# ashual/scene_generation

Hardware: AMD Instinct MI355X
Metric: images/sec G+D step, 128x128 <=8-obj scene graphs (higher is better)
Workload: dtype f32

## Files before the change

### scene_generation_amd/csrc/common.h

```cpp
#pragma once
#include <hip/hip_runtime.h>
#include <stdint.h>
#include <stdio.h>
#include <atomic>
#include "../../include/sg2im_hip.h"

#define SG_WAVE 64

void sg_set_error(const char* fmt, ...);
int sg_check_indices_if_enabled(const int64_t* idx, int64_t n, int64_t lo, int64_t hi, const char* what, hipStream_t s);

#define SG_ARG_CHECK(cond, ...)                 \
  do {                                          \
    if (!(cond)) {                              \
      sg_set_error(__VA_ARGS__);                \
      return -1;                                \
    }                                           \
  } while (0)

#define SG_LAUNCH_CHECK(name)                                               \
  do {                                                                      \
    hipError_t e__ = hipGetLastError();                                     \
    if (e__ != hipSuccess) {                                                \
      sg_set_error("%s: launch failed: %s", name, hipGetErrorString(e__)); \
      return (int)e__;                                                      \
    }                                                                       \
  } while (0)

enum SgOpt {
  SG_OPT_TILE,
  SG_OPT_T128_MIN,
  SG_OPT_TILE3,
  SG_OPT_TILE3_MIN,
  SG_OPT_SPLIT_TARGET,
  SG_OPT_SPLIT_KMIN,
  SG_OPT_SPLITS,
  SG_OPT_FIXEDTAP,
  SG_OPT_WINO_WT,
  SG_OPT_W24_SMALL,
  SG_OPT_W24_S,
  SG_OPT_W24_PMIN,
  SG_OPT_WINO_ADJOINT,
  SG_OPT_WINO24,
  SG_OPT_LINEAR_NSUB,
  SG_OPT_LINEAR_SKINNY,
  SG_OPT_WGRAD_ROWSUM,
  SG_OPT_LAYOUT_REG,
  SG_OPT_LAYOUT_DSPLIT,
  SG_OPT_BN_BLOCKS,
  SG_OPT_INSTNORM_REG,
  SG_OPT_WGRAD_XCD,
  SG_OPT_WINO_REUSE,
  SG_OPT_WINO_FOLD_CELLS,
  SG_OPT_WINO_PIPE,
  SG_OPT_CHECK_INDICES,
  SG_OPT_LAST_BLOCK,
  SG_OPT_WINO_GEMM_TILE,
  SG_OPT_WINO43,
  SG_OPT_GCONV_FUSED_GATHER,
  SG_OPT_W24_GEMM_TILE,
  SG_OPT_WINO_IN_FUSE,
  SG_OPT_W43_NSUB,
  SG_OPT_W43_KFOLD,
  SG_OPT_WAVE_PRIO,
  SG_OPT_PAR_XCD_CHUNK,
  SG_OPT_W43_TAIL_SPLIT,
  SG_OPT_TAIL_SMAX,
  SG_OPT_TAIL_KTMIN,
  SG_OPT_W43_WGRAD_TILE,
  SG_OPT_PAR_SPLIT,
  SG_OPT_TAIL_CAPTURE,
  SG_OPT_WGRAD_PADDED,
  SG_OPT_COUNT
};
extern std::atomic<int> g_sg_opt[SG_OPT_COUNT];
static inline int sg_opt(int id) { return g_sg_opt[id].load(std::memory_order_relaxed); }
extern FILE* g_sg_launch_log;

enum {
  SG_K_IGEMM_BASE = 0, SG_K_IGEMM_COUNT = 48,
  SG_K_LINEAR = 48, SG_K_LAYOUT_FWD, SG_K_LAYOUT_BWD, SG_K_INSTNORM, SG_K_BATCHNORM, SG_K_ADAM, SG_K_SEGSUM,
  SG_K_CROP, SG_K_OTHER,
  SG_K_WINO_GEMM_128, SG_K_WINO_GEMM_64, SG_K_WINO_XFORM,
  SG_K_HEAD,
  SG_K_INSTNORM_BWD,
  SG_K_WINO24_GEMM,
  SG_K_WINO43_GEMM,
  SG_K_LAYOUT_TEST_PLANES,
  SG_K_DEPROCESS,
  SG_K_LAYOUT_RGB,
  SG_K_KMEANS_ASSIGN, SG_K_KMEANS_UPDATE, SG_K_KMEANS_RELOCATE, SG_K_KMEANS_PP,
  SG_K_SCENEGRAPH_CENTERS, SG_K_SCENEGRAPH_DERIVE, SG_K_SCENEGRAPH_AGREE,
  SG_K_MAXPOOL3S2, SG_K_ADD_RELU, SG_K_BN_FOLD, SG_K_SGD, SG_K_CLASSIFY_STATS,
  SG_K_RECT_CONV_T64, SG_K_RECT_CONV_T32, SG_K_RECT_CONV_T64W, SG_K_RECT_REDUCE, SG_K_INCEPTION_POOL, SG_K_RESIZE_BILINEAR,
  SG_K_SOFTMAX_ROWS, SG_K_INCEPTION_SCORE,
  SG_K_COUNT
};
static inline int sg_igemm_kind(int family, int KS, int tile) {
  const int k = KS == 1 ? 0 : (KS == 3 ? 1 : (KS == 4 ? 2 : 3));
  return SG_K_IGEMM_BASE + family * 16 + k * 4 + tile;
}
extern int g_sg_prof_on;
void sg_prof_begin(int kind, hipStream_t s);
void sg_prof_end(int kind, hipStream_t s, double flops, double bytes);

struct SgProfScope {
  int kind; hipStream_t s; double flops, bytes; bool on;
  SgProfScope(int k, hipStream_t st, double f, double b) : kind(k), s(st), flops(f), bytes(b), on(g_sg_prof_on != 0) {
    if (on) sg_prof_begin(kind, s);
  }
  ~SgProfScope() { if (on) sg_prof_end(kind, s, flops, bytes); }
};

struct FastDiv {
  unsigned m, s, d;
  FastDiv() : m(0), s(0), d(1) {}
  explicit FastDiv(unsigned dd) : m(0), s(0), d(dd) {
    if (dd > 1) {
      unsigned sh = 0;
      while ((1u << sh) < dd) ++sh;
      m = (unsigned)((((uint64_t)1) << (31 + sh)) / dd + 1);
      s = sh - 1;
    }
  }
  __device__ __forceinline__ unsigned div(unsigned n) const { return d == 1 ? n : (__umulhi(n, m) >> s); }
};

static inline int sg_cdiv(int64_t a, int64_t b) { return (int)((a + b - 1) / b); }

__device__ __forceinline__ float sg_apply_act(float v, int act, float slope) {
  switch (act) {
    case SG_ACT_RELU: return v > 0.f ? v : 0.f;
    case SG_ACT_LEAKY: return v > 0.f ? v : v * slope;
    case SG_ACT_TANH: return tanhf(v);
    case SG_ACT_SIGMOID: return 1.f / (1.f + expf(-v));
    default: return v;
  }
}

__device__ __forceinline__ float sg_wave_sum(float v) {
#pragma unroll
  for (int o = 32; o > 0; o >>= 1) v += __shfl_xor(v, o, 64);
  return v;
}

__device__ __forceinline__ float sg_sum_strided(const float* __restrict__ p, size_t stride, int S) {
  float v = 0.f;
  for (int z0 = 0; z0 < S; z0 += 8) {
    float t[8];
#pragma unroll
    for (int e = 0; e < 8; ++e) t[e] = z0 + e < S ? p[(size_t)(z0 + e) * stride] : 0.f;
#pragma unroll
    for (int e = 0; e < 8; ++e)
      if (z0 + e < S) v += t[e];
  }
  return v;
}

__device__ __forceinline__ void sg_publish(float* p, float v) { __hip_atomic_store(p, v, __ATOMIC_RELAXED, __HIP_MEMORY_SCOPE_AGENT); }
__device__ __forceinline__ float sg_consume(const float* p) {
  return __hip_atomic_load(const_cast<float*>(p), __ATOMIC_RELAXED, __HIP_MEMORY_SCOPE_AGENT);
}
__device__ __forceinline__ bool sg_arrive_last(int* counter, int narrive, int* flag) {
  asm volatile("s_waitcnt vmcnt(0)" ::: "memory");
  __syncthreads();
  if (threadIdx.x == 0 && threadIdx.y == 0 && threadIdx.z == 0) {
    const int t = __hip_atomic_fetch_add(counter, 1, __ATOMIC_RELAXED, __HIP_MEMORY_SCOPE_AGENT);
    const int last = t == narrive - 1;
    if (last) __hip_atomic_store(counter, 0, __ATOMIC_RELAXED, __HIP_MEMORY_SCOPE_AGENT);
    *flag = last;
  }
  __syncthreads();
  return *flag != 0;
}
int* sg_counter_alloc(hipStream_t s, int n = 1, bool always = false, int family = 1);
float* sg_tail_scratch(hipStream_t s, size_t bytes);

__device__ __forceinline__ float sg_block_sum(float v, float* red) {
  const int lane = threadIdx.x & 63, wid = threadIdx.x >> 6, nw = (blockDim.x + 63) >> 6;
  v = sg_wave_sum(v);
  __syncthreads();
  if (lane == 0) red[wid] = v;
  __syncthreads();
  float t = 0.f;
  for (int i = 0; i < nw; ++i) t += red[i];
  return t;
}
```

### scene_generation_amd/csrc/layout.hip

```cpp
#include "common.h"
#include <stdlib.h>

namespace {

__device__ __forceinline__ float lin01(int j, int n) {
  if (n == 1) return 0.f;
  const float step = 1.f / (float)(n - 1);
  return j < n / 2 ? step * (float)j : 1.f - step * (float)(n - 1 - j);
}
__device__ __forceinline__ float lin10(int j, int n) {
  if (n == 1) return 1.f;
  const float step = -1.f / (float)(n - 1);
  return j < n / 2 ? 1.f + step * (float)j : 0.f - step * (float)(n - 1 - j);
}

struct Tap { int i0, i1; float w0, w1; };

__device__ __forceinline__ float tap_coord(float g, int size, int ac) {
  return ac ? (g + 1.f) * 0.5f * (float)(size - 1) : ((g + 1.f) * (float)size - 1.f) * 0.5f;
}
__device__ __forceinline__ Tap make_tap(float g, int size, int ac = 0) {
  Tap t;
  const float p = tap_coord(g, size, ac);
  if (!(fabsf(p) < 1e8f)) {
// ... 510 lines not shown
  const int max_fit = (int)(budget / per_obj);
  SG_ARG_CHECK(max_fit >= 1, "sg_masks_to_layout_fwd: D=%d too large for LDS", D);
  if (cap > max_fit) cap = max_fit;
  const size_t lds_bytes = (size_t)cap * per_obj;
  SgProfScope prof(SG_K_LAYOUT_FWD, s, 0, 4.0 * N * D * (double)H * W + 4.0 * O * D + (masks_i64 ? 8.0 : 4.0) * O * M * M);
  const int regform = sg_opt(SG_OPT_LAYOUT_REG);
  if (regform && use_vec == 4 && (size_t)D * 12 * sizeof(float) <= 64 * 1024) {
    const int tiles = sg_cdiv(H * W, 1024);
    int dsplit = sg_opt(SG_OPT_LAYOUT_DSPLIT);
    dsplit = dsplit < 1 ? 1 : (dsplit > 8 ? 8 : dsplit);
    if (dsplit > D / 16) dsplit = D / 16 > 0 ? D / 16 : 1;
    const int dchunk = sg_cdiv(D, dsplit);
    const dim3 g4(tiles, N, sg_cdiv(D, dchunk));
    const size_t lds = (size_t)dchunk * 12 * sizeof(float);
    if (masks_i64) hipLaunchKernelGGL((layout_fwd_reg_kernel<true, 12>), g4, dim3(256), lds, s, vecs, boxes, masks, seg_off, out, D, M, H, W, avg, g_align_corners, dchunk);
    else hipLaunchKernelGGL((layout_fwd_reg_kernel<false, 12>), g4, dim3(256), lds, s, vecs, boxes, masks, seg_off, out, D, M, H, W, avg, g_align_corners, dchunk);
    SG_LAUNCH_CHECK("sg_masks_to_layout_fwd");
    return 0;
  }
  const dim3 grid(sg_cdiv(H * W, 256 * use_vec), N);
#define LAUNCH_LAYOUT(I64, VEC)                                                                                         \
  do {                                                                                                                 \
    hipFuncSetAttribute(reinterpret_cast<const void*>(&layout_fwd_kernel<I64, VEC>),                                    \
                        hipFuncAttributeMaxDynamicSharedMemorySize, (int)lds_bytes);                                    \
    hipLaunchKernelGGL((layout_fwd_kernel<I64, VEC>), grid, dim3(256), lds_bytes, s, vecs, boxes, masks, seg_off, out, \
                       D, M, H, W, avg, cap, g_align_corners);                                                          \
  } while (0)
  if (masks_i64) { if (use_vec == 4) LAUNCH_LAYOUT(true, 4); else LAUNCH_LAYOUT(true, 1); }
  else { if (use_vec == 4) LAUNCH_LAYOUT(false, 4); else LAUNCH_LAYOUT(false, 1); }
#undef LAUNCH_LAYOUT
  SG_LAUNCH_CHECK("sg_masks_to_layout_fwd");
  return 0;
}

extern "C" size_t sg_masks_to_layout_test_ws_bytes(int O) { return (size_t)(O > 0 ? O : 1) * (sizeof(double) + sizeof(int32_t)) + 16; }

extern "C" int sg_masks_to_layout_test_fwd(const float* vecs, const float* boxes, const void* masks, int masks_i64,
                                           const int32_t* seg_off, float* out, void* ws, size_t ws_bytes, int N, int O, int D,
                                           int M, int H, int W, int avg, sgStream stream) {
  SG_ARG_CHECK(vecs && boxes && masks && seg_off && out && ws && N > 0 && O > 0 && D > 0 && M > 0 && H > 0 && W > 0,
               "sg_masks_to_layout_test_fwd: bad arguments");
  SG_ARG_CHECK(ws_bytes >= sg_masks_to_layout_test_ws_bytes(O), "sg_masks_to_layout_test_fwd: workspace too small");
  hipStream_t s = (hipStream_t)stream;
  double* mass = reinterpret_cast<double*>(ws);
  int32_t* order = reinterpret_cast<int32_t*>(mass + O);
  SgProfScope prof(SG_K_LAYOUT_FWD, s, 0, 4.0 * N * D * (double)H * W);
  const dim3 grid(sg_cdiv(H * W, 256), N);
  if (masks_i64) {
    hipLaunchKernelGGL((layout_mass_kernel<true>), dim3(O), dim3(256), 0, s, vecs, boxes, masks, mass, D, M, H, W, g_align_corners);
    hipLaunchKernelGGL(layout_order_kernel, dim3(N), dim3(64), 0, s, (const double*)mass, seg_off, order);
    hipLaunchKernelGGL((layout_test_fwd_kernel<true>), grid, dim3(256), 0, s, vecs, boxes, masks, seg_off,
                       (const int32_t*)order, out, D, M, H, W, avg, g_align_corners);
  } else {
    hipLaunchKernelGGL((layout_mass_kernel<false>), dim3(O), dim3(256), 0, s, vecs, boxes, masks, mass, D, M, H, W, g_align_corners);
    hipLaunchKernelGGL(layout_order_kernel, dim3(N), dim3(64), 0, s, (const double*)mass, seg_off, order);
    hipLaunchKernelGGL((layout_test_fwd_kernel<false>), grid, dim3(256), 0, s, vecs, boxes, masks, seg_off,
                       (const int32_t*)order, out, D, M, H, W, avg, g_align_corners);
  }
  SG_LAUNCH_CHECK("sg_masks_to_layout_test_fwd");
  return 0;
}

extern "C" size_t sg_masks_to_layout_test_planes_ws_bytes(int O) { return sg_masks_to_layout_test_ws_bytes(O); }

extern "C" int sg_masks_to_layout_test_planes(const float* vecs, const float* boxes, const void* masks, int masks_i64,
                                              const int32_t* seg_off, const int64_t* plane_idx, float* Z, int32_t* winner,
                                              float* value, void* ws, size_t ws_bytes, int N, int O, int D, int J, int M, int H,
                                              int W, int avg, sgStream stream) {
  SG_ARG_CHECK(vecs && boxes && masks && seg_off && plane_idx && Z && winner && ws && N > 0 && O > 0 && D > 0 && J > 0 && M > 0 &&
                   H > 0 && W > 0,
               "sg_masks_to_layout_test_planes: bad arguments");
  SG_ARG_CHECK(ws_bytes >= sg_masks_to_layout_test_planes_ws_bytes(O), "sg_masks_to_layout_test_planes: workspace too small");
  hipStream_t s = (hipStream_t)stream;
  double* mass = reinterpret_cast<double*>(ws);
  int32_t* order = reinterpret_cast<int32_t*>(mass + O);
  const int ac = g_align_corners;
  SgProfScope prof(SG_K_LAYOUT_TEST_PLANES, s, 0, 4.0 * N * (J + (value ? 2 : 1)) * (double)H * W);
  if (masks_i64) hipLaunchKernelGGL((layout_mass_kernel<true>), dim3(O), dim3(256), 0, s, vecs, boxes, masks, mass, D, M, H, W, ac);
  else hipLaunchKernelGGL((layout_mass_kernel<false>), dim3(O), dim3(256), 0, s, vecs, boxes, masks, mass, D, M, H, W, ac);
  hipLaunchKernelGGL(layout_order_kernel, dim3(N), dim3(64), 0, s, (const double*)mass, seg_off, order);
#define LAUNCH_PLANES(I64, VEC)                                                                                              \
  hipLaunchKernelGGL((layout_test_planes_kernel<I64, VEC>), dim3(sg_cdiv(H * W, 256 * VEC), N), dim3(256), 0, s, boxes, masks, \
                     seg_off, (const int32_t*)order, plane_idx, Z, winner, value, J, M, H, W, avg, ac)
  if (W % 4 == 0) { if (masks_i64) LAUNCH_PLANES(true, 4); else LAUNCH_PLANES(false, 4); }
  else { if (masks_i64) LAUNCH_PLANES(true, 1); else LAUNCH_PLANES(false, 1); }
#undef LAUNCH_PLANES
  SG_LAUNCH_CHECK("sg_masks_to_layout_test_planes");
  return 0;
}

extern "C" int sg_masks_to_layout_bwd_vecs(const float* gout, const float* boxes, const void* masks, int masks_i64,
                                           const int64_t* obj_to_img, const int32_t* seg_off, float* g_vecs, int N, int O,
                                           int D, int M, int H, int W, int avg, int d_begin, sgStream stream) {
  SG_ARG_CHECK(gout && boxes && masks && seg_off && g_vecs && N > 0 && O > 0 && D > 0 && d_begin >= 0 && d_begin < D,
               "sg_masks_to_layout_bwd_vecs: bad arguments");
  (void)obj_to_img;
  hipStream_t s = (hipStream_t)stream;
  if (d_begin > 0)
    hipLaunchKernelGGL(zero_cols_kernel, dim3(sg_cdiv((size_t)O * d_begin, 256)), dim3(256), 0, s, g_vecs, O, D, d_begin);
  SgProfScope prof(SG_K_LAYOUT_BWD, s, 0, 4.0 * N * (D - d_begin) * (double)H * W);
  const dim3 grid(D - d_begin, N);
  if (masks_i64) hipLaunchKernelGGL(layout_bwd_vecs_kernel<true>, grid, dim3(256), 0, s, gout, boxes, masks, seg_off, g_vecs, D, M, H, W, avg, d_begin, g_align_corners);
  else hipLaunchKernelGGL(layout_bwd_vecs_kernel<false>, grid, dim3(256), 0, s, gout, boxes, masks, seg_off, g_vecs, D, M, H, W, avg, d_begin, g_align_corners);
  SG_LAUNCH_CHECK("sg_masks_to_layout_bwd_vecs");
  return 0;
}

extern "C" int sg_crop_bbox_fwd(const float* feats, const float* boxes, const int64_t* box_to_feat, float* out, int N, int C,
                                int H, int W, int B, int HH, int WW, sgStream stream) {
  SG_ARG_CHECK(feats && N > 0 && C > 0 && B >= 0 && HH > 0 && WW > 0 && (B == 0 || (boxes && box_to_feat && out)),
               "sg_crop_bbox_fwd: bad arguments");
  if (B == 0) return 0;
  hipStream_t s = (hipStream_t)stream;
  SgProfScope prof(SG_K_CROP, s, 0, 4.0 * B * C * (double)HH * WW + 4.0 * N * C * (double)H * W);
  hipLaunchKernelGGL(crop_fwd_kernel, dim3(sg_cdiv((size_t)B * HH * WW, 256)), dim3(256), 0, s, feats, boxes, box_to_feat, out,
                     C, H, W, B, HH, WW, g_align_corners);
  SG_LAUNCH_CHECK("sg_crop_bbox_fwd");
  return 0;
}

extern "C" int sg_crop_bbox_bwd(const float* gout, const float* boxes, const int64_t* box_to_feat, float* g_feats, int N, int C,
                                int H, int W, int B, int HH, int WW, sgStream stream) {
  SG_ARG_CHECK(g_feats && N > 0 && C > 0 && H > 0 && W > 0 && B >= 0 && (B == 0 || (gout && boxes && box_to_feat)),
               "sg_crop_bbox_bwd: bad arguments");
  hipStream_t s = (hipStream_t)stream;
  if (B == 0) {
    if (hipMemsetAsync(g_feats, 0, (size_t)N * C * H * W * sizeof(float), s) != hipSuccess) {
      sg_set_error("sg_crop_bbox_bwd: hipMemsetAsync failed");
      return -1;
    }
    return 0;
  }
  SgProfScope prof(SG_K_CROP, s, 0, 4.0 * B * C * (double)HH * WW + 4.0 * N * C * (double)H * W);
  if (C <= 1)
    hipLaunchKernelGGL(crop_bwd_gather_kernel<1>, dim3(sg_cdiv(H * W, 256), N), dim3(256), 0, s, gout, boxes, box_to_feat,
                       g_feats, C, H, W, B, HH, WW, g_align_corners);
  else
    hipLaunchKernelGGL(crop_bwd_gather_kernel<4>, dim3(sg_cdiv(H * W, 256), N), dim3(256), 0, s, gout, boxes, box_to_feat,
                       g_feats, C, H, W, B, HH, WW, g_align_corners);
  SG_LAUNCH_CHECK("sg_crop_bbox_bwd");
  return 0;
}

struct JJTap { int i0, i1; float w0, w1; };
__device__ __forceinline__ JJTap jj_tap(float c0, float c1, int j, int n, int size) {
  const float X = (lin10(j, n) * c0 + lin01(j, n) * c1) * (float)size;
  const float hi = (float)(size - 1);
  const float f0 = fminf(fmaxf(floorf(X), 0.f), hi), f1 = fminf(fmaxf(f0 + 1.f, 0.f), hi);
  JJTap t;
  t.i0 = (int)f0; t.i1 = (int)f1; t.w0 = f1 - X; t.w1 = X - f0;
  return t;
}
__global__ void crop_jj_fwd_kernel(const float* __restrict__ feats, const float* __restrict__ boxes, float* __restrict__ out, int N,
                                   int C, int H, int W, int HH, int WW) {
  const size_t i = (size_t)blockIdx.x * blockDim.x + threadIdx.x;
  if (i >= (size_t)N * C * HH * WW) return;
  const int x = i % WW, y = (i / WW) % HH, c = (i / ((size_t)WW * HH)) % C, n = i / ((size_t)WW * HH * C);
  const JJTap tx = jj_tap(boxes[n * 4 + 0], boxes[n * 4 + 2], x, WW, W), ty = jj_tap(boxes[n * 4 + 1], boxes[n * 4 + 3], y, HH, H);
  const float* f = feats + ((size_t)n * C + c) * H * W;
  float v = (tx.w0 * ty.w0) * f[ty.i0 * W + tx.i0];
  v += (tx.w0 * ty.w1) * f[ty.i1 * W + tx.i0];
  v += (tx.w1 * ty.w0) * f[ty.i0 * W + tx.i1];
  v += (tx.w1 * ty.w1) * f[ty.i1 * W + tx.i1];
  out[i] = v;
}
__global__ void crop_jj_bwd_kernel(const float* __restrict__ gout, const float* __restrict__ boxes, float* __restrict__ gf, int N,
                                   int C, int H, int W, int HH, int WW) {
  const size_t i = (size_t)blockIdx.x * blockDim.x + threadIdx.x;
  if (i >= (size_t)N * C * H * W) return;
  const int u = i % W, r = (i / W) % H, c = (i / ((size_t)W * H)) % C, n = i / ((size_t)W * H * C);
  const float bx0 = boxes[n * 4 + 0], by0 = boxes[n * 4 + 1], bx1 = boxes[n * 4 + 2], by1 = boxes[n * 4 + 3];
  const float* g = gout + ((size_t)n * C + c) * HH * WW;
  float acc = 0.f;
  for (int y = 0; y < HH; ++y) {
    const JJTap ty = jj_tap(by0, by1, y, HH, H);
    const float wy = (ty.i0 == r ? ty.w0 : 0.f) + (ty.i1 == r ? ty.w1 : 0.f);
    if (ty.i0 != r && ty.i1 != r) continue;
    for (int x = 0; x < WW; ++x) {
      const JJTap tx = jj_tap(bx0, bx1, x, WW, W);
      if (tx.i0 != u && tx.i1 != u) continue;
      const float wx = (tx.i0 == u ? tx.w0 : 0.f) + (tx.i1 == u ? tx.w1 : 0.f);
      acc += (wx * wy) * g[y * WW + x];
    }
  }
  gf[i] = acc;
}

extern "C" int sg_crop_bbox_jj_fwd(const float* feats, const float* boxes, float* out, int N, int C, int H, int W, int HH, int WW,
                                   sgStream stream) {
  SG_ARG_CHECK(feats && boxes && out && N > 0 && C > 0 && H > 0 && W > 0 && HH > 0 && WW > 0, "sg_crop_bbox_jj_fwd: bad arguments");
  hipLaunchKernelGGL(crop_jj_fwd_kernel, dim3(sg_cdiv((size_t)N * C * HH * WW, 256)), dim3(256), 0, (hipStream_t)stream, feats, boxes,
                     out, N, C, H, W, HH, WW);
  SG_LAUNCH_CHECK("sg_crop_bbox_jj_fwd");
  return 0;
}
extern "C" int sg_crop_bbox_jj_bwd(const float* gout, const float* boxes, float* g_feats, int N, int C, int H, int W, int HH, int WW,
                                   sgStream stream) {
  SG_ARG_CHECK(gout && boxes && g_feats && N > 0 && C > 0 && H > 0 && W > 0 && HH > 0 && WW > 0, "sg_crop_bbox_jj_bwd: bad arguments");
  hipLaunchKernelGGL(crop_jj_bwd_kernel, dim3(sg_cdiv((size_t)N * C * H * W, 256)), dim3(256), 0, (hipStream_t)stream, gout, boxes,
                     g_feats, N, C, H, W, HH, WW);
  SG_LAUNCH_CHECK("sg_crop_bbox_jj_bwd");
  return 0;
}

extern "C" int sg_vector_pool_exchange(float* pool, const float* vectors, const int32_t* plan, float* out, int O, int R,
                                       int pool_size, sgStream stream) {
  SG_ARG_CHECK(pool && vectors && plan && out && O >= 0 && R > 0 && pool_size > 0, "sg_vector_pool_exchange: bad arguments");
  if (O == 0) return 0;
  hipStream_t s = (hipStream_t)stream;
  const dim3 grid(sg_cdiv((size_t)O * R, 256));
  hipLaunchKernelGGL(pool_gather_kernel, grid, dim3(256), 0, s, (const float*)pool, vectors, plan, out, O, R, pool_size);
  hipLaunchKernelGGL(pool_scatter_kernel, grid, dim3(256), 0, s, pool, vectors, plan, O, R, pool_size);
  SG_LAUNCH_CHECK("sg_vector_pool_exchange");
  return 0;
}

namespace {

__global__ void factored_weights_fwd_kernel(const float* __restrict__ W, const float* __restrict__ repr,
                                            const int64_t* __restrict__ objs, const int32_t* __restrict__ seg, float* __restrict__ wimg,
                                            int N, int M, int L, int KS2, int C, int R, int C2) {
  const size_t i = (size_t)blockIdx.x * blockDim.x + threadIdx.x;
  if (i >= (size_t)N * M * L * KS2) return;
  const int t = (int)(i % KS2);
  const int j = (int)((i / KS2) % L);
  const int m = (int)((i / ((size_t)KS2 * L)) % M);
  const int n = (int)(i / ((size_t)KS2 * L * M));
  const int cnt = seg[n + 1] - seg[n];
  const int Ct = C + R + C2;
  const float* Wm = W + (size_t)m * Ct * KS2 + t;
  float v = 0.f;
  if (j < cnt) {
    const int o = seg[n] + j;
    v = Wm[(size_t)objs[o] * KS2];
    const float* r = repr + (size_t)o * R;
    for (int d = 0; d < R; ++d) v += r[d] * Wm[(size_t)(C + d) * KS2];
  } else if (j < cnt + C2) {
    v = Wm[(size_t)(C + R + (j - cnt)) * KS2];
  }
  wimg[i] = v;
}

__global__ void factored_weights_bwd_w_kernel(const float* __restrict__ gwimg, const float* __restrict__ repr,
                                              const int64_t* __restrict__ objs, const int32_t* __restrict__ seg,
                                              const int64_t* __restrict__ img_idx, float* __restrict__ gW, int N, int O, int M,
                                              int L, int KS2, int C, int R, int C2) {
  const int Ct = C + R + C2;
  const size_t i = (size_t)blockIdx.x * blockDim.x + threadIdx.x;
  if (i >= (size_t)M * Ct * KS2) return;
  const int t = (int)(i % KS2);
  const int c = (int)((i / KS2) % Ct);
  const int m = (int)(i / ((size_t)KS2 * Ct));
  float s = 0.f;
  if (c < C + R) {
    for (int o = 0; o < O; ++o) {
      float wgt;
      if (c < C) { if ((int)objs[o] != c) continue; wgt = 1.f; }
      else wgt = repr[(size_t)o * R + (c - C)];
      const int n = (int)img_idx[o], j = o - seg[n];
      s += wgt * gwimg[(((size_t)n * M + m) * L + j) * KS2 + t];
    }
  } else {
    const int e = c - C - R;
    for (int n = 0; n < N; ++n) s += gwimg[(((size_t)n * M + m) * L + (seg[n + 1] - seg[n]) + e) * KS2 + t];
  }
  gW[i] = s;
}

__global__ void __launch_bounds__(256) factored_weights_bwd_w_lds_kernel(
    const float* __restrict__ gwimg, const float* __restrict__ repr, const int64_t* __restrict__ objs,
    const int32_t* __restrict__ seg, const int64_t* __restrict__ img_idx, float* __restrict__ gW, int N, int O, int M, int L,
    int KS2, int C, int R, int C2) {
  extern __shared__ int ws_lds[];
  int* cls = ws_lds;
  int* base = ws_lds + O;
  for (int o = threadIdx.x; o < O; o += 256) {
    const int n = (int)img_idx[o];
    cls[o] = (int)objs[o];
    base[o] = n * M * L + (o - seg[n]);
  }
  __syncthreads();
  const int Ct = C + R + C2;
  const size_t i = (size_t)blockIdx.x * blockDim.x + threadIdx.x;
  if (i >= (size_t)M * Ct * KS2) return;
  const int t = (int)(i % KS2);
  const int c = (int)((i / KS2) % Ct);
  const int m = (int)(i / ((size_t)KS2 * Ct));
  const int mL = m * L;
  float s = 0.f;
  if (c < C) {
    for (int o = 0; o < O; ++o)
      if (cls[o] == c) s += gwimg[(size_t)(base[o] + mL) * KS2 + t];
  } else if (c < C + R) {
    const float* rp = repr + (c - C);
#pragma unroll 4
    for (int o = 0; o < O; ++o) s += rp[(size_t)o * R] * gwimg[(size_t)(base[o] + mL) * KS2 + t];
  } else {
    const int e = c - C - R;
    for (int n = 0; n < N; ++n) s += gwimg[(((size_t)n * M + m) * L + (seg[n + 1] - seg[n]) + e) * KS2 + t];
  }
  gW[i] = s;
}

__global__ void __launch_bounds__(256) factored_weights_bwd_repr_kernel(const float* __restrict__ gwimg, const float* __restrict__ W,
                                                                       const int32_t* __restrict__ seg,
                                                                       const int64_t* __restrict__ img_idx,
                                                                       float* __restrict__ grepr, int O, int M, int L, int KS2,
                                                                       int C, int R, int C2) {
  const int w = blockIdx.x * 4 + (threadIdx.x >> 6), lane = threadIdx.x & 63;
  if (w >= O * R) return;
  const int o = w / R, d = w - o * R;
  const int n = (int)img_idx[o], j = o - seg[n];
  const int Ct = C + R + C2;
  float s = 0.f;
  for (int q = lane; q < M * KS2; q += 64) {
    const int m = q / KS2, t = q - m * KS2;
    s += gwimg[(((size_t)n * M + m) * L + j) * KS2 + t] * W[((size_t)m * Ct + C + d) * KS2 + t];
  }
  s = sg_wave_sum(s);
  if (lane == 0) grepr[w] = s;
}

}

extern "C" int sg_factored_weights_fwd(const float* w, const float* repr, const int64_t* objs, const int32_t* seg_off,
                                       float* wimg, int N, int O, int M, int L, int KS2, int C, int R, int C2, sgStream stream) {
  SG_ARG_CHECK(w && repr && objs && seg_off && wimg && N > 0 && O >= 0 && M > 0 && L > 0 && KS2 > 0 && C >= 0 && R >= 0 && C2 >= 0,
               "sg_factored_weights_fwd: bad arguments");
  const size_t n = (size_t)N * M * L * KS2;
  hipLaunchKernelGGL(factored_weights_fwd_kernel, dim3(sg_cdiv(n, 256)), dim3(256), 0, (hipStream_t)stream, w, repr, objs, seg_off,
                     wimg, N, M, L, KS2, C, R, C2);
  SG_LAUNCH_CHECK("sg_factored_weights_fwd");
  return 0;
}

extern "C" int sg_factored_weights_bwd(const float* gwimg, const float* w, const float* repr, const int64_t* objs,
                                       const int32_t* seg_off, const int64_t* img_idx, float* gw, float* grepr, int N, int O,
                                       int M, int L, int KS2, int C, int R, int C2, sgStream stream) {
  SG_ARG_CHECK(gwimg && w && repr && objs && seg_off && img_idx && (gw || grepr) && N > 0 && O > 0,
               "sg_factored_weights_bwd: bad arguments");
  hipStream_t s = (hipStream_t)stream;
  if (gw) {
    const size_t n = (size_t)M * (C + R + C2) * KS2;
    if (O <= 4096 && (size_t)N * M * L < (1u << 30))
      hipLaunchKernelGGL(factored_weights_bwd_w_lds_kernel, dim3(sg_cdiv(n, 256)), dim3(256), (size_t)O * 2 * sizeof(int), s, gwimg,
                         repr, objs, seg_off, img_idx, gw, N, O, M, L, KS2, C, R, C2);
    else
      hipLaunchKernelGGL(factored_weights_bwd_w_kernel, dim3(sg_cdiv(n, 256)), dim3(256), 0, s, gwimg, repr, objs, seg_off, img_idx,
                         gw, N, O, M, L, KS2, C, R, C2);
  }
  if (grepr && R > 0)
    hipLaunchKernelGGL(factored_weights_bwd_repr_kernel, dim3(sg_cdiv((size_t)O * R, 4)), dim3(256), 0, s, gwimg, w, seg_off, img_idx,
                       grepr, O, M, L, KS2, C, R, C2);
  SG_LAUNCH_CHECK("sg_factored_weights_bwd");
  return 0;
}

namespace {

__global__ void __launch_bounds__(256) layout_objmap_kernel(const float* __restrict__ gout, const float* __restrict__ vecs,
                                                           const int64_t* __restrict__ o2i, const int32_t* __restrict__ seg,
                                                           float* __restrict__ T, int D, int HW, int avg) {
  const int o = blockIdx.y;
  const int px = blockIdx.x * 256 + threadIdx.x;
  if (px >= HW) return;
  const int n = (int)o2i[o];
  const float* g = gout + (size_t)n * D * HW + px;
  const float* v = vecs + (size_t)o * D;
  float s = 0.f;
  for (int d = 0; d < D; ++d) s += g[(size_t)d * HW] * v[d];
  if (avg) { const int cnt = seg[n + 1] - seg[n]; s = s / (float)(cnt > 1 ? cnt : 1); }
  T[(size_t)o * HW + px] = s;
}

__device__ __forceinline__ void layout_axis_range(float b0, float b1, int n_pix, int M, int y, int& lo, int& hi, int ac) {
  const float p0 = tap_coord(box_coord(0.f, b0, b1), M, ac), p1 = tap_coord(box_coord(1.f, b0, b1), M, ac);
  lo = 0; hi = n_pix - 1;
  if (n_pix == 1 || !(fabsf(p0) < 1e8f) || !(fabsf(p1) < 1e8f)) return;
  const float s = (p1 - p0) / (float)(n_pix - 1);
  if (fabsf(s) < 1e-6f) return;
  float a = ((float)(y - 1) - p0) / s, b = ((float)(y + 1) - p0) / s;
  if (a > b) { const float t = a; a = b; b = t; }
  const float fl = floorf(a) - 1.f, fh = ceilf(b) + 1.f;
  lo = fl < 0.f ? 0 : (fl > (float)(n_pix - 1) ? n_pix : (int)fl);
  hi = fh > (float)(n_pix - 1) ? n_pix - 1 : (fh < 0.f ? -1 : (int)fh);
}

__global__ void __launch_bounds__(256) layout_bwd_masks_kernel(const float* __restrict__ T, const float* __restrict__ boxes,
                                                              float* __restrict__ gm, int M, int H, int W, int ac) {
  const int o = blockIdx.y;
  const int e = blockIdx.x * 256 + threadIdx.x;
  if (e >= M * M) return;
  const int y = e / M, x = e - y * M;
  const float x0 = boxes[o * 4 + 0], y0 = boxes[o * 4 + 1], x1 = boxes[o * 4 + 2], y1 = boxes[o * 4 + 3];
  int hlo, hhi, wlo, whi;
  layout_axis_range(y0, y1, H, M, y, hlo, hhi, ac);
  layout_axis_range(x0, x1, W, M, x, wlo, whi, ac);
  const float* t = T + (size_t)o * H * W;
  float s = 0.f;
  for (int h = hlo; h <= hhi; ++h) {
    const Tap ty = make_tap(box_coord(lin01(h, H), y0, y1), M, ac);
    const float wy = (ty.i0 == y ? ty.w0 : 0.f) + (ty.i1 == y ? ty.w1 : 0.f);
    if (wy == 0.f) continue;
    for (int w = wlo; w <= whi; ++w) {
      const Tap tx = make_tap(box_coord(lin01(w, W), x0, x1), M, ac);
      const float wx = (tx.i0 == x ? tx.w0 : 0.f) + (tx.i1 == x ? tx.w1 : 0.f);
      if (wx != 0.f) s += t[h * W + w] * (wy * wx);
    }
  }
  gm[(size_t)o * M * M + e] = s;
}

template <bool I64>
__global__ void __launch_bounds__(256) layout_bwd_boxes_kernel(const float* __restrict__ T, const float* __restrict__ boxes,
                                                              const void* __restrict__ masks, float* __restrict__ gb, int M, int H,
                                                              int W, int ac) {
  __shared__ float red[16];
  const size_t o = blockIdx.x;
  const float x0 = boxes[o * 4 + 0], y0 = boxes[o * 4 + 1], x1 = boxes[o * 4 + 2], y1 = boxes[o * 4 + 3];
  const float dx = x1 - x0, dy = y1 - y0;
  const float scale = ac ? 0.5f * (float)(M - 1) : 0.5f * (float)M;
  const float* t = T + o * H * W;
  float g0 = 0.f, g1 = 0.f, g2 = 0.f, g3 = 0.f;
  for (int p = threadIdx.x; p < H * W; p += 256) {
    const int h = p / W, w = p - h * W;
    const float Y = lin01(h, H), X = lin01(w, W);
    const Tap ty = make_tap(box_coord(Y, y0, y1), M, ac), tx = make_tap(box_coord(X, x0, x1), M, ac);
    const float m00 = mask_at<I64>(masks, o, M, ty.i0, tx.i0), m01 = mask_at<I64>(masks, o, M, ty.i0, tx.i1);
    const float m10 = mask_at<I64>(masks, o, M, ty.i1, tx.i0), m11 = mask_at<I64>(masks, o, M, ty.i1, tx.i1);
    const float px = tap_coord(box_coord(X, x0, x1), M, ac), py = tap_coord(box_coord(Y, y0, y1), M, ac);
    const bool fin = fabsf(px) < 1e8f && fabsf(py) < 1e8f;
    const float flx = floorf(px), fly = floorf(py);
    const float ix0 = (flx >= 0.f && flx < (float)M) ? 1.f : 0.f, ix1 = (flx + 1.f >= 0.f && flx + 1.f < (float)M) ? 1.f : 0.f;
    const float iy0 = (fly >= 0.f && fly < (float)M) ? 1.f : 0.f, iy1 = (fly + 1.f >= 0.f && fly + 1.f < (float)M) ? 1.f : 0.f;
    const float dSdx = ((m01 * ix1 - m00 * ix0) * ty.w0 + (m11 * ix1 - m10 * ix0) * ty.w1);
    const float dSdy = ((m10 * iy1 - m00 * iy0) * tx.w0 + (m11 * iy1 - m01 * iy0) * tx.w1);
    const float tv = fin ? t[p] : 0.f;
    const float cx = tv * dSdx * scale * 2.f / (dx * dx), cy = tv * dSdy * scale * 2.f / (dy * dy);
    g0 += cx * (X - x1); g2 += -cx * (X - x0);
    g1 += cy * (Y - y1); g3 += -cy * (Y - y0);
  }
  g0 = sg_block_sum(g0, red); g1 = sg_block_sum(g1, red); g2 = sg_block_sum(g2, red); g3 = sg_block_sum(g3, red);
  if (threadIdx.x == 0) { gb[o * 4 + 0] = g0; gb[o * 4 + 1] = g1; gb[o * 4 + 2] = g2; gb[o * 4 + 3] = g3; }
}

}

extern "C" size_t sg_masks_to_layout_bwd_geom_ws_bytes(int O, int H, int W) { return (size_t)(O > 0 ? O : 1) * H * W * sizeof(float); }

extern "C" int sg_masks_to_layout_bwd_geom(const float* gout, const float* vecs, const float* boxes, const void* masks, int masks_i64,
                                           const int64_t* obj_to_img, const int32_t* seg_off, float* g_masks, float* g_boxes,
                                           void* ws, size_t ws_bytes, int N, int O, int D, int M, int H, int W, int avg,
                                           sgStream stream) {
  SG_ARG_CHECK(gout && vecs && boxes && masks && obj_to_img && seg_off && ws && (g_masks || g_boxes) && N > 0 && O > 0 && D > 0,
               "sg_masks_to_layout_bwd_geom: bad arguments");
  SG_ARG_CHECK(ws_bytes >= sg_masks_to_layout_bwd_geom_ws_bytes(O, H, W), "sg_masks_to_layout_bwd_geom: workspace too small");
  SG_ARG_CHECK(!(g_masks && masks_i64), "sg_masks_to_layout_bwd_geom: integer masks have no gradient");
  hipStream_t s = (hipStream_t)stream;
  float* T = reinterpret_cast<float*>(ws);
  hipLaunchKernelGGL(layout_objmap_kernel, dim3(sg_cdiv(H * W, 256), O), dim3(256), 0, s, gout, vecs, obj_to_img, seg_off, T, D, H * W, avg);
  if (g_masks)
    hipLaunchKernelGGL(layout_bwd_masks_kernel, dim3(sg_cdiv(M * M, 256), O), dim3(256), 0, s, (const float*)T, boxes, g_masks, M, H, W,
                       g_align_corners);
  if (g_boxes) {
    if (masks_i64) hipLaunchKernelGGL(layout_bwd_boxes_kernel<true>, dim3(O), dim3(256), 0, s, (const float*)T, boxes, masks, g_boxes, M, H, W, g_align_corners);
    else hipLaunchKernelGGL(layout_bwd_boxes_kernel<false>, dim3(O), dim3(256), 0, s, (const float*)T, boxes, masks, g_boxes, M, H, W, g_align_corners);
  }
  SG_LAUNCH_CHECK("sg_masks_to_layout_bwd_geom");
  return 0;
}
```

### scene_generation_amd/csrc/runtime.hip

```cpp
#include "common.h"
#include <stdarg.h>
#include <mutex>
#include <vector>
#include <stdlib.h>
#include <string.h>
#include <ctype.h>

static thread_local char t_err[512] = "ok";

void sg_set_error(const char* fmt, ...) {
  va_list ap;
  va_start(ap, fmt);
  vsnprintf(t_err, sizeof(t_err), fmt, ap);
  va_end(ap);
}

extern "C" const char* sg_last_error_string(void) { return t_err; }
extern "C" int sg_version(void) { return 100; }

int g_sg_prof_on = 0;

std::atomic<int> g_sg_opt[SG_OPT_COUNT];
FILE* g_sg_launch_log = nullptr;
namespace {
struct OptDef { const char* name; int def; };
const OptDef kOpts[SG_OPT_COUNT] = {
    {"tile", -1}, {"t128_min", 384}, {"tile3", 1}, {"tile3_min", 768}, {"split_target", 1536}, {"split_kmin", 2048}, {"splits", -1}, {"fixedtap", 1}, {"wino_wt", 1},
    {"w24_small", 1}, {"w24_s", -1}, {"w24_pmin", 256}, {"wino_adjoint", 1}, {"wino24", 1}, {"linear_nsub", 2},
    {"linear_skinny", 2048}, {"wgrad_rowsum", 1}, {"layout_reg", 1}, {"layout_dsplit", 1}, {"bn_blocks", 4096},
    {"instnorm_reg", 2}, {"wgrad_xcd", 1}, {"wino_reuse", 1}, {"wino_fold_cells", 1}, {"wino_pipe", 2},
    {"check_indices", 0}, {"last_block", 0}, {"wino_gemm_tile", 0}, {"wino43", 1}, {"gconv_fused_gather", 1}, {"w24_gemm_tile", 2}, {"wino_in_fuse", 1}, {"w43_nsub", 1}, {"w43_kfold", 256}, {"wave_prio", 0}, {"par_xcd_chunk", 16}, {"w43_tail_split", 2}, {"tail_smax", 4}, {"tail_ktmin", 8}, {"w43_wgrad_tile", 0}, {"par_split", 1}, {"tail_capture", 1}, {"wgrad_padded", 1}};
struct OptInit {
  OptInit() {
    for (int i = 0; i < SG_OPT_COUNT; ++i) {
      char env[64] = "SG_";
      size_t n = 3;
      for (const char* c = kOpts[i].name; *c && n + 1 < sizeof(env); ++c) env[n++] = (char)toupper((unsigned char)*c);
      env[n] = 0;
      const char* e = getenv(env);
      g_sg_opt[i].store((e && *e) ? atoi(e) : kOpts[i].def, std::memory_order_relaxed);
    }
    const char* lf = getenv("SG_LAUNCH_LOG");
    if (lf && *lf) g_sg_launch_log = fopen(lf, "a");
  }
} g_opt_init;
int opt_index(const char* key) {
  if (!key) return -1;
  for (int i = 0; i < SG_OPT_COUNT; ++i)
    if (strcmp(key, kOpts[i].name) == 0) return i;
  return -1;
}
}

extern "C" int sg_num_options(void) { return SG_OPT_COUNT; }
extern "C" const char* sg_option_name(int i) { return (i >= 0 && i < SG_OPT_COUNT) ? kOpts[i].name : nullptr; }
extern "C" int sg_option_default(int i) { return (i >= 0 && i < SG_OPT_COUNT) ? kOpts[i].def : 0; }
extern "C" int sg_get_option(const char* key, int* value) {
  const int i = opt_index(key);
  if (i < 0 || !value) { sg_set_error("sg_get_option: unknown option '%s'", key ? key : "(null)"); return -1; }
  *value = sg_opt(i);
  return 0;
}
extern "C" int sg_set_option(const char* key, int value) {
  const int i = opt_index(key);
  if (i < 0) { sg_set_error("sg_set_option: unknown option '%s'", key ? key : "(null)"); return -1; }
  g_sg_opt[i].store(value, std::memory_order_relaxed);
  return 0;
}

namespace {
constexpr int CNT_RING = 65536, CNT_CAPTURED = 262144, CNT_DEVICES = 16;
std::mutex g_cnt_mu;
int* g_cnt_pool[CNT_DEVICES] = {};
unsigned g_cnt_ring[CNT_DEVICES] = {};
int g_cnt_cap[CNT_DEVICES] = {};
}

int* sg_counter_alloc(hipStream_t s, int n, bool always, int family) {
  if ((!always && !(sg_opt(SG_OPT_LAST_BLOCK) & family)) || n < 1 || n > 4096) return nullptr;
  int dev = 0;
  if (hipGetDevice(&dev) != hipSuccess || dev < 0 || dev >= CNT_DEVICES) return nullptr;
  hipStreamCaptureStatus cap = hipStreamCaptureStatusNone;
  const bool capturing = hipStreamIsCapturing(s, &cap) == hipSuccess && cap != hipStreamCaptureStatusNone;
  std::lock_guard<std::mutex> lk(g_cnt_mu);
  if (!g_cnt_pool[dev]) {
    if (capturing) return nullptr;
    int* p = nullptr;
    const size_t bytes = (size_t)(CNT_RING + CNT_CAPTURED) * sizeof(int);
    if (hipMalloc((void**)&p, bytes) != hipSuccess) return nullptr;
    if (hipMemset(p, 0, bytes) != hipSuccess) { hipFree(p); return nullptr; }
    g_cnt_pool[dev] = p;
  }
  if (capturing) {
    if (g_cnt_cap[dev] + n > CNT_CAPTURED) return nullptr;
    int* r = g_cnt_pool[dev] + CNT_RING + g_cnt_cap[dev];
    g_cnt_cap[dev] += n;
    return r;
  }
  unsigned at = g_cnt_ring[dev];
  if (at + (unsigned)n > (unsigned)CNT_RING) at = 0;
  g_cnt_ring[dev] = at + (unsigned)n;
  return g_cnt_pool[dev] + at;
}

namespace {
struct TailScratch { int dev; hipStream_t s; float* p; size_t bytes; };
std::vector<TailScratch> g_tail;
}

namespace {
struct TailCap { float* p; size_t bytes; };
TailCap g_tail_cap[CNT_DEVICES] = {};
void tail_cap_reserve(int dev, size_t bytes) {
  if (dev < 0 || dev >= CNT_DEVICES || g_tail_cap[dev].bytes >= bytes) return;
  float* q = nullptr;
  if (hipMalloc((void**)&q, bytes) != hipSuccess) return;
  g_tail_cap[dev].p = q; g_tail_cap[dev].bytes = bytes;
}
}

float* sg_tail_scratch(hipStream_t s, size_t bytes) {
  int dev = 0;
  if (hipGetDevice(&dev) != hipSuccess) return nullptr;
  hipStreamCaptureStatus cap = hipStreamCaptureStatusNone;
  const bool capturing = hipStreamIsCapturing(s, &cap) == hipSuccess && cap != hipStreamCaptureStatusNone;
  std::lock_guard<std::mutex> lk(g_cnt_mu);
  if (capturing)
    return (sg_opt(SG_OPT_TAIL_CAPTURE) && dev >= 0 && dev < CNT_DEVICES && g_tail_cap[dev].bytes >= bytes) ? g_tail_cap[dev].p : nullptr;
  tail_cap_reserve(dev, bytes);
  for (auto& t : g_tail)
    if (t.dev == dev && t.s == s) {
      if (t.bytes >= bytes) return t.p;
      float* q = nullptr;
      if (hipMalloc((void**)&q, bytes) != hipSuccess) return nullptr;
      t.p = q; t.bytes = bytes;
      return q;
    }
  float* q = nullptr;
  if (hipMalloc((void**)&q, bytes) != hipSuccess) return nullptr;
  g_tail.push_back(TailScratch{dev, s, q, bytes});
  return q;
}

namespace {
struct Rec { int kind; hipEvent_t e0, e1; double flops, bytes; };
std::mutex g_mu;
std::vector<Rec> g_recs;
std::vector<hipEvent_t> g_free;
hipEvent_t g_open[SG_K_COUNT];
double g_ms[SG_K_COUNT], g_flops[SG_K_COUNT], g_bytes[SG_K_COUNT];
int64_t g_cnt[SG_K_COUNT];
const char* kTail[SG_K_COUNT - SG_K_IGEMM_COUNT] = {"linear", "layout_fwd", "layout_bwd", "instnorm", "batchnorm", "adam",
                                                    "segsum", "crop", "other", "wino_bgemm_t128", "wino_bgemm_t64",
                                                    "wino_transforms", "head_conv", "instnorm_bwd", "wino24_bgemm_t128", "wino43_bgemm_t64",
                                                    "layout_test_planes", "deprocess", "layout_rgb", "kmeans_assign", "kmeans_update",
                                                    "kmeans_relocate", "kmeans_pp", "scenegraph_centers", "scenegraph_derive",
                                                    "scenegraph_agree", "maxpool3s2", "add_relu", "bn_fold", "sgd", "classify_stats",
                                                    "rect_conv_t64", "rect_conv_t32", "rect_conv_t64x128", "rect_reduce", "inception_pool",
                                                    "resize_bilinear", "softmax_rows", "inception_score"};
char g_names[SG_K_COUNT][32];
bool g_names_init = false;
void init_names() {
  if (g_names_init) return;
  const char* fam[3] = {"kn0", "kn1", "nk"};
  const int ks[4] = {1, 3, 4, 7};
  const char* tl[4] = {"128", "64", "32", "64x128"};
  for (int f = 0; f < 3; ++f)
    for (int k = 0; k < 4; ++k)
      for (int t = 0; t < 4; ++t)
        snprintf(g_names[f * 16 + k * 4 + t], 32, "igemm_%s_k%d_t%s", fam[f], ks[k], tl[t]);
  for (int i = SG_K_IGEMM_COUNT; i < SG_K_COUNT; ++i) snprintf(g_names[i], 32, "%s", kTail[i - SG_K_IGEMM_COUNT]);
  g_names_init = true;
}

hipEvent_t get_event() {
  if (!g_free.empty()) { hipEvent_t e = g_free.back(); g_free.pop_back(); return e; }
  hipEvent_t e;
  hipEventCreate(&e);
  return e;
}

void drain() {
  for (auto& r : g_recs) {
    hipEventSynchronize(r.e1);
    float ms = 0.f;
    hipEventElapsedTime(&ms, r.e0, r.e1);
    g_ms[r.kind] += ms; g_flops[r.kind] += r.flops; g_bytes[r.kind] += r.bytes; g_cnt[r.kind] += 1;
    g_free.push_back(r.e0); g_free.push_back(r.e1);
  }
  g_recs.clear();
}
}

void sg_prof_begin(int kind, hipStream_t s) {
  std::lock_guard<std::mutex> lk(g_mu);
  hipEvent_t e = get_event();
  hipEventRecord(e, s);
  g_open[kind] = e;
}

void sg_prof_end(int kind, hipStream_t s, double flops, double bytes) {
  std::lock_guard<std::mutex> lk(g_mu);
  hipEvent_t e = get_event();
  hipEventRecord(e, s);
  g_recs.push_back(Rec{kind, g_open[kind], e, flops, bytes});
  if (g_recs.size() > 8192) drain();
}

extern "C" int sg_prof_enable(int on) { g_sg_prof_on = on; return 0; }
extern "C" int sg_prof_reset(void) {
  std::lock_guard<std::mutex> lk(g_mu);
  drain();
  for (int i = 0; i < SG_K_COUNT; ++i) { g_ms[i] = g_flops[i] = g_bytes[i] = 0; g_cnt[i] = 0; }
  return 0;
}
extern "C" int sg_prof_num_kinds(void) { return SG_K_COUNT; }
extern "C" const char* sg_prof_kind_name(int kind) {
  init_names();
  return (kind >= 0 && kind < SG_K_COUNT) ? g_names[kind] : "?";
}
extern "C" int sg_prof_read(int kind, double* total_ms, int64_t* launches, double* flops, double* bytes) {
  if (kind < 0 || kind >= SG_K_COUNT) { sg_set_error("sg_prof_read: bad kind %d", kind); return -1; }
  std::lock_guard<std::mutex> lk(g_mu);
  drain();
  if (total_ms) *total_ms = g_ms[kind];
  if (launches) *launches = g_cnt[kind];
  if (flops) *flops = g_flops[kind];
  if (bytes) *bytes = g_bytes[kind];
  return 0;
}
```

Baseline: 1137.

## Split factored-weights backward into LDS-tiled appearance GEMM and class-list kernels

Replaces the single per-element factored weight-gradient kernel with two kernels. One stages chunks of gathered gwimg and repr rows in LDS and accumulates a 4-wide register tile per thread, so global data is reused for the appearance/repr columns. The other builds per-class linked lists of objects in LDS, so each class column sums only its own objects rather than scanning every object. This adds extra launches, LDS staging and list-building overhead, and keeps the old path behind an option.

```diff
diff --git a/scene_generation_amd/csrc/common.h b/scene_generation_amd/csrc/common.h
--- a/scene_generation_amd/csrc/common.h
+++ b/scene_generation_amd/csrc/common.h
@@ -71,6 +71,7 @@
   SG_OPT_PAR_SPLIT,
   SG_OPT_TAIL_CAPTURE,
   SG_OPT_WGRAD_PADDED,
+  SG_OPT_FACTORED_TILED,
   SG_OPT_COUNT
 };
 extern std::atomic<int> g_sg_opt[SG_OPT_COUNT];
diff --git a/scene_generation_amd/csrc/layout.hip b/scene_generation_amd/csrc/layout.hip
--- a/scene_generation_amd/csrc/layout.hip
+++ b/scene_generation_amd/csrc/layout.hip
@@ -836,6 +836,165 @@
   gW[i] = s;
 }
 
+constexpr int FT_MAX_KS2 = 256, FT_CHUNK = 128, FT_CHUNK_BYTES = 40960, FT_PARTS = 16;
+inline int ft_dqw(int KS2) { const int q = 256 / KS2; return q > 16 ? 16 : q; }
+inline int ft_chunk(int KS2) {
+  int oc = FT_CHUNK;
+  while ((size_t)oc * (KS2 + 4 * ft_dqw(KS2)) * sizeof(float) > FT_CHUNK_BYTES) oc >>= 1;
+  return oc;
+}
+__device__ __forceinline__ void ft_stage_base(int* base, const int32_t* __restrict__ seg, const int64_t* __restrict__ img_idx, int O,
+                                              int ML, int tid) {
+  for (int o = tid; o < O; o += 256) {
+    const int n = (int)img_idx[o];
+    base[o] = n * ML + (o - seg[n]);
+  }
+}
+__global__ void __launch_bounds__(256) factored_weights_bwd_w_app_kernel(
+    const float* __restrict__ gwimg, const float* __restrict__ repr, const int32_t* __restrict__ seg,
+    const int64_t* __restrict__ img_idx, float* __restrict__ gW, int O, int M, int L, int KS2, int C, int R, int C2, int dqw, int oc) {
+  extern __shared__ int ft_lds[];
+  int* base = ft_lds;
+  const int Op = (O + 3) & ~3;
+  const int tid = threadIdx.x, m = blockIdx.y;
+  const int Ct = C + R + C2, mL = m * L;
+  ft_stage_base(base, seg, img_idx, O, M * L, tid);
+  const int dw = 4 * dqw, d0 = (int)blockIdx.x * dw;
+  float* gl = reinterpret_cast<float*>(ft_lds + Op);
+  float* rl = gl + (size_t)oc * KS2;
+  const int t = tid % KS2, dq = tid / KS2;
+  const bool live = dq < dqw && d0 + 4 * dq < R;
+  const bool vec_g = (KS2 & 3) == 0 && (reinterpret_cast<uintptr_t>(gwimg) & 15) == 0;
+  const bool vec_r = (R & 3) == 0 && (reinterpret_cast<uintptr_t>(repr) & 15) == 0;
+  float a0 = 0.f, a1 = 0.f, a2 = 0.f, a3 = 0.f;
+  for (int o0 = 0; o0 < O; o0 += oc) {
+    const int no = O - o0 < oc ? O - o0 : oc;
+    __syncthreads();
+    if (vec_g) {
+      const int q4 = KS2 >> 2;
+#pragma unroll 4
+      for (int e = tid; e < no * q4; e += 256) {
+        const int oi = e / q4, q = e - oi * q4;
+        reinterpret_cast<float4*>(gl)[e] = *reinterpret_cast<const float4*>(gwimg + (size_t)(base[o0 + oi] + mL) * KS2 + 4 * q);
+      }
+    } else {
+#pragma unroll 8
+      for (int e = tid; e < no * KS2; e += 256) {
+        const int oi = e / KS2, tt = e - oi * KS2;
+        gl[e] = gwimg[(size_t)(base[o0 + oi] + mL) * KS2 + tt];
+      }
+    }
+    if (vec_r) {
+#pragma unroll 4
+      for (int e = tid; e < no * dqw; e += 256) {
+        const int oi = e / dqw, q = e - oi * dqw;
+        float4 v = make_float4(0.f, 0.f, 0.f, 0.f);
+        if (d0 + 4 * q < R) v = *reinterpret_cast<const float4*>(repr + (size_t)(o0 + oi) * R + d0 + 4 * q);
+        reinterpret_cast<float4*>(rl)[e] = v;
+      }
+    } else {
+#pragma unroll 8
+      for (int e = tid; e < no * dw; e += 256) {
+        const int oi = e / dw, dd = e - oi * dw;
+        rl[e] = d0 + dd < R ? repr[(size_t)(o0 + oi) * R + d0 + dd] : 0.f;
+      }
+    }
+    __syncthreads();
+    if (live) {
+      const float* gp = gl + t;
+      const float* rp = rl + 4 * dq;
+#pragma unroll 4
+      for (int oi = 0; oi < no; ++oi) {
+        const float g = gp[oi * KS2];
+        const float4 r = *reinterpret_cast<const float4*>(rp + oi * dw);
+        a0 += r.x * g; a1 += r.y * g; a2 += r.z * g; a3 += r.w * g;
+      }
+    }
+  }
+  if (live) {
+    const int d = d0 + 4 * dq;
+    float* out = gW + ((size_t)m * Ct + C + d) * KS2 + t;
+    out[0] = a0;
+    if (d + 1 < R) out[KS2] = a1;
+    if (d + 2 < R) out[2 * (size_t)KS2] = a2;
+    if (d + 3 < R) out[3 * (size_t)KS2] = a3;
+  }
+}
+__global__ void __launch_bounds__(256) factored_weights_bwd_w_cls_kernel(
+    const float* __restrict__ gwimg, const int64_t* __restrict__ objs, const int32_t* __restrict__ seg,
+    const int64_t* __restrict__ img_idx, float* __restrict__ gW, int N, int O, int M, int L, int KS2, int C, int R, int C2) {
+  extern __shared__ int ft_lds[];
+  int* base = ft_lds;
+  int* cls = base + O;
+  int* nxt = cls + O;
+  int* pfirst = nxt + O;
+  int* plast = pfirst + 256;
+  int* head = plast + 256;
+  int* cntl = head + 256;
+  const int tid = threadIdx.x, m = blockIdx.y;
+  const int Ct = C + R + C2, mL = m * L;
+  const int x0 = (int)blockIdx.x * 256;
+  const int c_lo = x0 / KS2;
+  int c_hi = (x0 + 255) / KS2;
+  if (c_hi > C - 1) c_hi = C - 1;
+  const int Wc = c_hi - c_lo + 1;
+  ft_stage_base(base, seg, img_idx, O, M * L, tid);
+  for (int o = tid; o < O; o += 256) cls[o] = (int)objs[o];
+  if ((x0 + 255) / KS2 >= C)
+    for (int n = tid; n < N; n += 256) cntl[n] = seg[n + 1] - seg[n];
+  __syncthreads();
+  int P = Wc > 0 ? 256 / Wc : 0;
+  if (P > FT_PARTS) P = FT_PARTS;
+  if (tid < Wc * P) {
+    const int k = tid % Wc, p = tid / Wc, c = c_lo + k;
+    const int len = (O + P - 1) / P, ob = p * len, oe = ob + len < O ? ob + len : O;
+    int first = -1, prev = -1;
+    for (int o = ob; o < oe; ++o)
+      if (cls[o] == c) {
+        if (prev < 0) first = o; else nxt[prev] = o;
+        prev = o;
+      }
+    pfirst[tid] = first;
+    plast[tid] = prev;
+  }
+  __syncthreads();
+  if (tid < Wc) {
+    int first = -1, tail = -1;
+    for (int p = 0; p < P; ++p) {
+      const int f = pfirst[p * Wc + tid];
+      if (f >= 0) {
+        if (tail < 0) first = f; else nxt[tail] = f;
+        tail = plast[p * Wc + tid];
+      }
+    }
+    if (tail >= 0) nxt[tail] = -1;
+    head[tid] = first;
+  }
+  __syncthreads();
+  const int x = x0 + tid;
+  if (x >= (C + C2) * KS2) return;
+  const int cp = x / KS2, t = x - cp * KS2;
+  float s = 0.f;
+  if (cp < C) {
+    for (int o = head[cp - c_lo]; o >= 0; o = nxt[o]) s += gwimg[(size_t)(base[o] + mL) * KS2 + t];
+    gW[((size_t)m * Ct + cp) * KS2 + t] = s;
+  } else {
+    const int e = cp - C;
+    const float* gp = gwimg + ((size_t)mL + e) * KS2 + t;
+    const size_t is = (size_t)M * L * KS2;
+    int n = 0;
+    for (; n + 8 <= N; n += 8) {
+      float v[8];
+#pragma unroll
+      for (int i = 0; i < 8; ++i) v[i] = gp[(n + i) * is + (size_t)cntl[n + i] * KS2];
+#pragma unroll
+      for (int i = 0; i < 8; ++i) s += v[i];
+    }
+    for (; n < N; ++n) s += gp[n * is + (size_t)cntl[n] * KS2];
+    gW[((size_t)m * Ct + C + R + e) * KS2 + t] = s;
+  }
+}
+
 __global__ void __launch_bounds__(256) factored_weights_bwd_repr_kernel(const float* __restrict__ gwimg, const float* __restrict__ W,
                                                                        const int32_t* __restrict__ seg,
                                                                        const int64_t* __restrict__ img_idx,
@@ -876,7 +1035,19 @@
   hipStream_t s = (hipStream_t)stream;
   if (gw) {
     const size_t n = (size_t)M * (C + R + C2) * KS2;
-    if (O <= 4096 && (size_t)N * M * L < (1u << 30))
+    const bool lds_ok = O <= 4096 && (size_t)N * M * L < (1u << 30);
+    if (lds_ok && sg_opt(SG_OPT_FACTORED_TILED) && KS2 <= FT_MAX_KS2 && M <= 65535 && N <= 4096) {
+      const int dqw = ft_dqw(KS2), oc = ft_chunk(KS2);
+      const int nA = R > 0 ? sg_cdiv(sg_cdiv(R, 4), dqw) : 0, nC = sg_cdiv((size_t)(C + C2) * KS2, 256);
+      const size_t lds_a = ((size_t)((O + 3) & ~3) + (size_t)oc * (KS2 + 4 * dqw)) * sizeof(int);
+      const size_t lds_c = ((size_t)3 * O + 768 + N) * sizeof(int);
+      if (nA > 0)
+        hipLaunchKernelGGL(factored_weights_bwd_w_app_kernel, dim3(nA, M), dim3(256), lds_a, s, gwimg, repr, seg_off, img_idx, gw, O, M,
+                           L, KS2, C, R, C2, dqw, oc);
+      if (nC > 0)
+        hipLaunchKernelGGL(factored_weights_bwd_w_cls_kernel, dim3(nC, M), dim3(256), lds_c, s, gwimg, objs, seg_off, img_idx, gw, N, O,
+                           M, L, KS2, C, R, C2);
+    } else if (lds_ok)
       hipLaunchKernelGGL(factored_weights_bwd_w_lds_kernel, dim3(sg_cdiv(n, 256)), dim3(256), (size_t)O * 2 * sizeof(int), s, gwimg,
                          repr, objs, seg_off, img_idx, gw, N, O, M, L, KS2, C, R, C2);
     else
diff --git a/scene_generation_amd/csrc/runtime.hip b/scene_generation_amd/csrc/runtime.hip
--- a/scene_generation_amd/csrc/runtime.hip
+++ b/scene_generation_amd/csrc/runtime.hip
@@ -29,7 +29,7 @@
     {"w24_small", 1}, {"w24_s", -1}, {"w24_pmin", 256}, {"wino_adjoint", 1}, {"wino24", 1}, {"linear_nsub", 2},
     {"linear_skinny", 2048}, {"wgrad_rowsum", 1}, {"layout_reg", 1}, {"layout_dsplit", 1}, {"bn_blocks", 4096},
     {"instnorm_reg", 2}, {"wgrad_xcd", 1}, {"wino_reuse", 1}, {"wino_fold_cells", 1}, {"wino_pipe", 2},
-    {"check_indices", 0}, {"last_block", 0}, {"wino_gemm_tile", 0}, {"wino43", 1}, {"gconv_fused_gather", 1}, {"w24_gemm_tile", 2}, {"wino_in_fuse", 1}, {"w43_nsub", 1}, {"w43_kfold", 256}, {"wave_prio", 0}, {"par_xcd_chunk", 16}, {"w43_tail_split", 2}, {"tail_smax", 4}, {"tail_ktmin", 8}, {"w43_wgrad_tile", 0}, {"par_split", 1}, {"tail_capture", 1}, {"wgrad_padded", 1}};
+    {"check_indices", 0}, {"last_block", 0}, {"wino_gemm_tile", 0}, {"wino43", 1}, {"gconv_fused_gather", 1}, {"w24_gemm_tile", 2}, {"wino_in_fuse", 1}, {"w43_nsub", 1}, {"w43_kfold", 256}, {"wave_prio", 0}, {"par_xcd_chunk", 16}, {"w43_tail_split", 2}, {"tail_smax", 4}, {"tail_ktmin", 8}, {"w43_wgrad_tile", 0}, {"par_split", 1}, {"tail_capture", 1}, {"wgrad_padded", 1}, {"factored_tiled", 1}};
 struct OptInit {
   OptInit() {
     for (int i = 0; i < SG_OPT_COUNT; ++i) {
```

Result: no change. 1138, median of 6 (+0.1%).
